# sonoisa/code2vec

Hardware: AMD Instinct MI355X
Metric: path_contexts_per_sec (higher is better)
Workload: dtype bf16; 1 GPU; model=code2vec-top11, global_batch=1024, seq_len=200, parallelism=dp1, terminal_vocab=360632, label_vocab=72416, embed=100, encode=100

## Files before the change

code2vec_amd/ops/csrc/bindings.cpp:

```cpp

#include <torch/extension.h>

#include <ATen/hip/HIPContext.h>
#include <c10/hip/HIPStream.h>
#include <hip/hip_runtime.h>

#include <map>

#define CHK(x) TORCH_CHECK(x, #x)
#define CHK_CONTIG(t) TORCH_CHECK((t).is_contiguous(), #t " must be contiguous")
#define CHK_CUDA(t) TORCH_CHECK((t).is_cuda(), #t " must be on GPU")
#define CHK_DT(t, dt) TORCH_CHECK((t).scalar_type() == dt, #t " dtype mismatch")

extern "C" {
void launch_gather_concat_fwd(const int*, const int*, const int*, const void*,
                              const void*, void*, long, int, int, int,
                              hipStream_t);
void launch_gather_concat_bwd(const int*, const int*, const int*, const void*,
                              float*, float*, long, int, int, hipStream_t);
void launch_embed_scatter_sorted(const int*, const long*, const void*, float*,
                                 void*, unsigned char*, long, long, int, int,
                                 int, int, int, hipStream_t);
void launch_embed_scatter_heavy(const int*, const long*, const int*,
                                const void*, float*, long, long, int, int,
                                int, int, int, hipStream_t);
void launch_adam_table_bf16(void*, const void*, const long*, int*, const int*,
                            float*, float*, float*, float*, long, int, long,
                            long, long, int, int, int, int, const double*,
                            float, float, float, float, float, int,
                            hipStream_t);
long group_tables_partials(long, long);
void launch_group_tables(const int*, const int*, const int*, long, int, int,
                         int*, int*, int*, int*, int*, int*, long*, int*,
                         long*, hipStream_t);
void launch_embed_scatter_heavy_pair(const int*, const long*, const int*,
                                     float*, int, const int*, const long*,
                                     const int*, float*, int, const void*,
                                     long, int, int, hipStream_t);
void launch_clear_i32_pair(int*, long, int*, long, hipStream_t);
void launch_count_indices(const int*, int*, long, hipStream_t);
void launch_cast_clear_rows(float*, const int*, unsigned char*, void*, long,
                            int, hipStream_t);
void launch_scatter_group(const int*, int*, int*, long*, long, hipStream_t);
void launch_exclusive_scan(const int*, int*, int*, long, hipStream_t);
size_t cub_exclusive_scan_temp_bytes(long);
void launch_cub_exclusive_scan(const int*, int*, void*, size_t, long,
                               hipStream_t);
void launch_combiner_fwd(const void*, const void*, const float*, const float*,
                         void*, void*, float*, float*, long, int, int, int,
                         float, unsigned long long,
                         const unsigned long long*, int, hipStream_t);
int launch_combiner_fwd_scores(const void*, const void*, const float*,
                               const float*, void*, void*, float*, float*,
                               long, int, int, int, float, unsigned long long,
                               const unsigned long long*, int, const float*,
                               float*, hipStream_t);
void launch_bump_u64(void*, unsigned long long, hipStream_t);
void launch_gather_combiner_fwd(const int*, const int*, const int*,
                                const void*, const void*, int, int,
                                const void*, const float*, const float*,
                                void*, void*, float*, float*, long, int, int,
                                int, float, unsigned long long,
                                const unsigned long long*, hipStream_t);
void launch_wgrad_gather(const int*, const int*, const int*, const void*,
                         const void*, int, int, const void*, float*, long,
                         int, int, int, hipStream_t);
void launch_combiner_bwd(const void*, const void*, const void*, const float*,
                         const float*, const float*, const float*, void*,
                         float*, float*, long, int, int, float, hipStream_t);
void launch_combiner_bwd_recompute(const float*, const float*, const void*,
                                   int, const float*, int, const void*,
                                   const void*, const float*, const float*,
                                   const float*, const float*, void*, float*,
                                   float*, long, int, float, hipStream_t);
void launch_attention_fwd(const void*, const float*, const int*, float*,
                          void*, float*, int, int, int, int, hipStream_t);
void launch_attention_bwd(const void*, int, const float*, const void*,
                          const float*, const int*, const float*, void*,
                          float*, float*, int, int, int, int, int,
                          hipStream_t);
int attention_stream_supported(int, int);
void launch_attention_fwd_scores(const void*, const float*, const int*,
                                 float*, void*, float*, int, int, int, int,
                                 hipStream_t);
void launch_attention_bwd_compact_reg(const void*, int, const float*,
                                      const void*, const int*, const float*,
                                      float*, float*, int, int, int, int, int,
                                      hipStream_t);
int attention_packed_chunk();
void launch_attention_packed_fwd(const void*, const float*, const int*,
                                 const int*, float*, void*, float*, long, long,
                                 int, int, hipStream_t);
void launch_attention_packed_bwd(const void*, int, const float*, const void*,
                                 const float*, const int*, const int*,
                                 const float*, void*, float*, int*, float*,
                                 long, long, int, int, hipStream_t);
void launch_combiner_bwd_recompute_packed(
    const float*, const float*, const void*, int, const float*, const int*,
    long, const void*, const void*, const float*, const float*, const float*,
    const float*, void*, float*, float*, long, int, float, hipStream_t);
void launch_slab_sum2_f32(const float*, const float*, float*, float*, int,
                          int, hipStream_t);
void launch_loss_reduce(const float*, float*, float*, int, hipStream_t);
void launch_wgrad_reduce(const float*, void*, int, int, int, hipStream_t);
void launch_lsm_nll_fwd(const void*, const long*, const float*, float*,
                        float*, int, long, hipStream_t);
void launch_lsm_nll_bwd(const void*, const long*, const float*, const float*,
                        const float*, const float*, void*, int, long,
                        hipStream_t);
bool launch_wgrad_pipe(const void*, const void*, float*, long, int, int, int,
                       int, hipStream_t);
void launch_wgrad(const void*, const void*, float*, long, int, int, int,
                  hipStream_t);
void launch_dgrad(const void*, const void*, void*, long, int, int,
                  hipStream_t);
void launch_head_wgrad(const void*, const void*, void*, long, long, int,
                       hipStream_t);
// ... 1257 lines not shown
  CHK_CUDA(sorted_idx); CHK_CONTIG(sorted_idx);
  CHK_DT(sorted_idx, torch::kInt32);
  CHK_DT(dtable, torch::kFloat32); CHK_CONTIG(dtable);
  TORCH_CHECK(dtable.dim() == 2, "dtable must be [T, S]");
  const long T = dtable.size(0);
  const int S = dtable.size(1);
  check_table_record(perm, counts, gout, T, S, M, KP, off0, off1);
  TORCH_CHECK(sorted_idx.numel() == perm.numel(), "sorted_idx/perm sizes");
  TORCH_CHECK(S % 2 == 0 && S <= 512 && KP % 2 == 0 && off0 % 2 == 0 &&
                  off1 % 2 == 0, "embed_scatter_heavy: S/KP/offset alignment");
  TORCH_CHECK(thr >= 32, "embed_scatter_heavy: thr must be >= 32");
  launch_embed_scatter_heavy(sorted_idx.data_ptr<int>(),
                             perm.data_ptr<long>(), counts.data_ptr<int>(),
                             gout.data_ptr(), dtable.data_ptr<float>(),
                             perm.numel(), M, (int)KP, S, (int)off0,
                             (int)off1, (int)thr, cur_stream());
}

static void adam_table_bf16_impl(
    torch::Tensor p, torch::Tensor gout, torch::Tensor perm,
    torch::Tensor counts, torch::Tensor cursor, torch::Tensor scratch,
    torch::Tensor master, torch::Tensor m, torch::Tensor v,
    torch::Tensor bc_pow, int64_t M, int64_t KP, int64_t off0, int64_t off1,
    int64_t thr, double lr, double b1, double b2, double eps, double wd,
    bool clear_counts) {
  CHK_CUDA(p); CHK_CONTIG(p); CHK_DT(p, torch::kBFloat16);
  TORCH_CHECK(p.dim() == 2, "p must be [T, S]");
  const long T = p.size(0);
  const int S = p.size(1);
  check_table_record(perm, counts, gout, T, S, M, KP, off0, off1);
  CHK_CONTIG(cursor); CHK_DT(cursor, torch::kInt32);
  TORCH_CHECK(cursor.numel() >= T, "cursor shorter than T");
  CHK_DT(scratch, torch::kFloat32); CHK_CONTIG(scratch);
  CHK_DT(master, torch::kFloat32); CHK_CONTIG(master);
  CHK_DT(m, torch::kFloat32); CHK_CONTIG(m);
  CHK_DT(v, torch::kFloat32); CHK_CONTIG(v);
  CHK_DT(bc_pow, torch::kFloat64);
  const long n = T * S;
  TORCH_CHECK(scratch.numel() == n && master.numel() == n &&
                  m.numel() == n && v.numel() == n, "state sizes");
  TORCH_CHECK(S % 4 == 0 && KP % 4 == 0 && off0 % 4 == 0 && off1 % 4 == 0,
              "adam_table_bf16: S, KP and offsets must be multiples of 4");
  TORCH_CHECK(n / 4 < (1L << 32), "adam_table_bf16: table too large");
  TORCH_CHECK(thr >= 32, "adam_table_bf16: thr must be >= 32");
  launch_adam_table_bf16(
      p.data_ptr(), gout.data_ptr(), perm.data_ptr<long>(),
      counts.data_ptr<int>(), cursor.data_ptr<int>(),
      scratch.data_ptr<float>(), master.data_ptr<float>(),
      m.data_ptr<float>(), v.data_ptr<float>(), T, S, counts.numel(),
      perm.numel(), M, (int)KP, (int)off0, (int)off1, (int)thr,
      (const double*)bc_pow.data_ptr(), (float)lr, (float)b1, (float)b2,
      (float)eps, (float)wd, clear_counts ? 1 : 0, cur_stream());
}

void adam_table_bf16(torch::Tensor p, torch::Tensor gout, torch::Tensor perm,
                     torch::Tensor counts, torch::Tensor cursor,
                     torch::Tensor scratch, torch::Tensor master,
                     torch::Tensor m, torch::Tensor v, torch::Tensor bc_pow,
                     int64_t M, int64_t KP, int64_t off0, int64_t off1,
                     int64_t thr, double lr, double b1, double b2, double eps,
                     double wd) {
  adam_table_bf16_impl(p, gout, perm, counts, cursor, scratch, master, m, v,
                       bc_pow, M, KP, off0, off1, thr, lr, b1, b2, eps, wd,
                       true);
}

void adam_table_bf16_keep_counts(
    torch::Tensor p, torch::Tensor gout, torch::Tensor perm,
    torch::Tensor counts, torch::Tensor cursor, torch::Tensor scratch,
    torch::Tensor master, torch::Tensor m, torch::Tensor v,
    torch::Tensor bc_pow, int64_t M, int64_t KP, int64_t off0, int64_t off1,
    int64_t thr, double lr, double b1, double b2, double eps, double wd) {
  adam_table_bf16_impl(p, gout, perm, counts, cursor, scratch, master, m, v,
                       bc_pow, M, KP, off0, off1, thr, lr, b1, b2, eps, wd,
                       false);
}


namespace {
struct GroupStream {
  hipStream_t side = nullptr;
  hipEvent_t ready = nullptr;
  hipEvent_t done = nullptr;
};
std::map<int, GroupStream>& group_streams() {
  static std::map<int, GroupStream> m;
  return m;
}
GroupStream& group_stream_for(int device) {
  auto& m = group_streams();
  auto it = m.find(device);
  if (it == m.end()) {
    GroupStream g;
    g.side = c10::hip::getStreamFromPool(false, device).stream();
    C10_HIP_CHECK(hipEventCreateWithFlags(&g.ready, hipEventDisableTiming));
    C10_HIP_CHECK(hipEventCreateWithFlags(&g.done, hipEventDisableTiming));
    it = m.emplace(device, g).first;
  }
  return it->second;
}
void check_i32(const torch::Tensor& t, long n, const char* what) {
  TORCH_CHECK(t.is_cuda() && t.is_contiguous() &&
                  t.scalar_type() == torch::kInt32 && t.numel() >= n,
              "group_tables: ", what, " must be contiguous int32 on the GPU "
              "with at least ", n, " elements");
}
}

bool group_tables(torch::Tensor starts, torch::Tensor paths,
                  torch::Tensor ends, torch::Tensor counts_t,
                  torch::Tensor counts_p, torch::Tensor cursor_t,
                  torch::Tensor cursor_p, torch::Tensor partial,
                  torch::Tensor sorted_t, torch::Tensor perm_t,
                  torch::Tensor sorted_p, torch::Tensor perm_p,
                  int64_t rows_t, int64_t rows_p, bool side_stream) {
  const long M = starts.numel();
  TORCH_CHECK(M > 0 && 2 * M < (1L << 31), "group_tables: bad entry count");
  TORCH_CHECK(rows_t > 0 && rows_p > 0 && rows_t < (1L << 31) &&
                  rows_p < (1L << 31), "group_tables: bad histogram length");
  check_i32(starts, M, "starts"); check_i32(paths, M, "paths");
  check_i32(ends, M, "ends");
  TORCH_CHECK(paths.numel() == M && ends.numel() == M,
              "group_tables: starts/paths/ends sizes differ");
  check_i32(counts_t, rows_t, "counts_t"); check_i32(counts_p, rows_p, "counts_p");
  check_i32(cursor_t, rows_t, "cursor_t"); check_i32(cursor_p, rows_p, "cursor_p");
  check_i32(partial, group_tables_partials(rows_t, rows_p), "partial");
  check_i32(sorted_t, 2 * M, "sorted_t"); check_i32(sorted_p, M, "sorted_p");
  CHK_CUDA(perm_t); CHK_CONTIG(perm_t); CHK_DT(perm_t, torch::kInt64);
  CHK_CUDA(perm_p); CHK_CONTIG(perm_p); CHK_DT(perm_p, torch::kInt64);
  TORCH_CHECK(perm_t.numel() >= 2 * M && perm_p.numel() >= M,
              "group_tables: perm buffers too short");

  auto cur = at::hip::getCurrentHIPStream();
  hipStream_t launch_on = cur.stream();
  bool on_side = false;
  GroupStream* gs = nullptr;
  if (side_stream) {
    hipStreamCaptureStatus cap = hipStreamCaptureStatusNone;
    C10_HIP_CHECK(hipStreamIsCapturing(cur.stream(), &cap));
    if (cap == hipStreamCaptureStatusNone) {
      gs = &group_stream_for(cur.device_index());
      C10_HIP_CHECK(hipEventRecord(gs->ready, cur.stream()));
      C10_HIP_CHECK(hipStreamWaitEvent(gs->side, gs->ready, 0));
      launch_on = gs->side;
      on_side = true;
    }
  }
  launch_group_tables(
      starts.data_ptr<int>(), paths.data_ptr<int>(), ends.data_ptr<int>(), M,
      (int)rows_t, (int)rows_p, counts_t.data_ptr<int>(),
      counts_p.data_ptr<int>(), cursor_t.data_ptr<int>(),
      cursor_p.data_ptr<int>(), partial.data_ptr<int>(),
      sorted_t.data_ptr<int>(), perm_t.data_ptr<long>(),
      sorted_p.data_ptr<int>(), perm_p.data_ptr<long>(), launch_on);
  if (on_side) C10_HIP_CHECK(hipEventRecord(gs->done, gs->side));
  return on_side;
}

void group_tables_wait() {
  auto cur = at::hip::getCurrentHIPStream();
  auto& m = group_streams();
  auto it = m.find(cur.device_index());
  TORCH_CHECK(it != m.end(), "group_tables_wait: no side-stream grouping");
  C10_HIP_CHECK(hipStreamWaitEvent(cur.stream(), it->second.done, 0));
}

int64_t group_tables_partials_len(int64_t rows_t, int64_t rows_p) {
  return group_tables_partials(rows_t, rows_p);
}

void embed_scatter_heavy_pair(torch::Tensor sorted_t, torch::Tensor perm_t,
                              torch::Tensor counts_t, torch::Tensor dtable_t,
                              torch::Tensor sorted_p, torch::Tensor perm_p,
                              torch::Tensor counts_p, torch::Tensor dtable_p,
                              torch::Tensor gout, int64_t M, int64_t KP,
                              int64_t thr) {
  CHK_DT(dtable_t, torch::kFloat32); CHK_CONTIG(dtable_t);
  CHK_DT(dtable_p, torch::kFloat32); CHK_CONTIG(dtable_p);
  TORCH_CHECK(dtable_t.dim() == 2 && dtable_p.dim() == 2,
              "dtable must be [T, S]");
  const int St = dtable_t.size(1), Sp = dtable_p.size(1);
  check_table_record(perm_t.narrow(0, 0, 2 * M), counts_t, gout,
                     dtable_t.size(0), St, M, KP, 0, St + Sp);
  check_table_record(perm_p.narrow(0, 0, M), counts_p, gout,
                     dtable_p.size(0), Sp, M, KP, St, St);
  check_i32(sorted_t, 2 * M, "sorted_t"); check_i32(sorted_p, M, "sorted_p");
  TORCH_CHECK(St % 2 == 0 && Sp % 2 == 0 && St <= 512 && Sp <= 512 &&
                  KP % 2 == 0, "embed_scatter_heavy_pair: S/KP alignment");
  TORCH_CHECK(thr >= 32, "embed_scatter_heavy_pair: thr must be >= 32");
  launch_embed_scatter_heavy_pair(
      sorted_t.data_ptr<int>(), perm_t.data_ptr<long>(),
      counts_t.data_ptr<int>(), dtable_t.data_ptr<float>(), St,
      sorted_p.data_ptr<int>(), perm_p.data_ptr<long>(),
      counts_p.data_ptr<int>(), dtable_p.data_ptr<float>(), Sp,
      gout.data_ptr(), M, (int)KP, (int)thr, cur_stream());
}

void clear_i32_pair(torch::Tensor a, torch::Tensor b) {
  check_i32(a, 0, "a"); check_i32(b, 0, "b");
  launch_clear_i32_pair(a.data_ptr<int>(), a.numel(), b.data_ptr<int>(),
                        b.numel(), cur_stream());
}

void adam_step_f32(torch::Tensor p, torch::Tensor g, torch::Tensor m,
                   torch::Tensor v, torch::Tensor bc_pow, double lr,
                   double b1, double b2, double eps, double wd) {
  CHK_CUDA(p); CHK_DT(p, torch::kFloat32); CHK_DT(g, torch::kFloat32);
  CHK_DT(bc_pow, torch::kFloat64);
  launch_adam_f32(p.data_ptr<float>(), g.data_ptr<float>(),
                  m.data_ptr<float>(), v.data_ptr<float>(), p.numel(),
                  (const double*)bc_pow.data_ptr(), (float)lr, (float)b1,
                  (float)b2, (float)eps, (float)wd, cur_stream());
}

void adam_step_f32_multi(std::vector<torch::Tensor> ps,
                         std::vector<torch::Tensor> gs,
                         std::vector<torch::Tensor> ms,
                         std::vector<torch::Tensor> vs,
                         torch::Tensor bc_pow, double lr, double b1,
                         double b2, double eps, double wd) {
  const int n = (int)ps.size();
  TORCH_CHECK(n >= 1 && n <= 8, "adam_step_f32_multi: 1..8 tensors");
  TORCH_CHECK((int)gs.size() == n && (int)ms.size() == n &&
              (int)vs.size() == n, "adam_step_f32_multi: list sizes");
  CHK_DT(bc_pow, torch::kFloat64);
  float* pp[8]; const float* gp[8]; float* mp[8]; float* vp[8]; long ns[8];
  for (int t = 0; t < n; ++t) {
    CHK_CUDA(ps[t]); CHK_CONTIG(ps[t]); CHK_DT(ps[t], torch::kFloat32);
    CHK_CONTIG(gs[t]); CHK_DT(gs[t], torch::kFloat32);
    TORCH_CHECK(ps[t].numel() == gs[t].numel() &&
                ps[t].numel() == ms[t].numel() &&
                ps[t].numel() == vs[t].numel(), "sizes");
    pp[t] = ps[t].data_ptr<float>();
    gp[t] = gs[t].data_ptr<float>();
    mp[t] = ms[t].data_ptr<float>();
    vp[t] = vs[t].data_ptr<float>();
    ns[t] = ps[t].numel();
  }
  launch_adam_f32_multi(pp, gp, mp, vp, ns, n,
                        (const double*)bc_pow.data_ptr(), (float)lr,
                        (float)b1, (float)b2, (float)eps, (float)wd,
                        cur_stream());
}

PYBIND11_MODULE(TORCH_EXTENSION_NAME, m) {
  m.def("gather_concat_fwd", &gather_concat_fwd);
  m.def("gather_concat_bwd", &gather_concat_bwd);
  m.def("embed_scatter_sorted", &embed_scatter_sorted);
  m.def("group_by_index", &group_by_index);
  m.def("cast_clear_rows", &cast_clear_rows);
  m.def("combiner_fwd", &combiner_fwd);
  m.def("gather_combiner_fwd", &gather_combiner_fwd);
  m.def("wgrad_gather", &wgrad_gather);
  m.def("combiner_bwd", &combiner_bwd);
  m.def("attention_fwd", &attention_fwd);
  m.def("attention_bwd", &attention_bwd);
  m.def("attention_fwd_cvb", &attention_fwd_cvb);
  m.def("attention_bwd_compact", &attention_bwd_compact);
  m.def("combiner_fwd_scores", &combiner_fwd_scores);
  m.def("attention_stream_ok", &attention_stream_ok);
  m.def("attention_fwd_scores", &attention_fwd_scores);
  m.def("attention_bwd_compact_reg", &attention_bwd_compact_reg);
  m.def("attention_pool_packed", &attention_pool_packed);
  m.def("combiner_bwd_recompute", &combiner_bwd_recompute);
  m.def("attention_packed_bwd_compact", &attention_packed_bwd_compact);
  m.def("attention_packed_bwd", &attention_packed_bwd);
  m.def("combiner_bwd_recompute_packed", &combiner_bwd_recompute_packed);
  m.def("slab_sum2_f32", &slab_sum2_f32);
  m.def("loss_reduce", &loss_reduce);
  m.def("wgrad_reduce", &wgrad_reduce);
  m.def("logsoftmax_nll_fwd", &logsoftmax_nll_fwd);
  m.def("logsoftmax_nll_bwd", &logsoftmax_nll_bwd);
  m.def("wgrad", &wgrad);
  m.def("wgrad_pipe", &wgrad_pipe);
  m.def("colsum_bf16", &colsum_bf16);
  m.def("head_fwd", &head_fwd);
  m.def("head_fwd_img", &head_fwd_img);
  m.def("swizzle_a", &swizzle_a);
  m.def("logsoftmax_nll_finalize", &logsoftmax_nll_finalize);
  m.def("lsm_partial", &lsm_partial);
  m.def("head_wgrad", &head_wgrad);
  m.def("head_dgrad", &head_dgrad);
  m.def("exclusive_scan", &exclusive_scan);
  m.def("cub_exclusive_scan", &cub_exclusive_scan);
  m.def("cub_scan_temp_bytes", &cub_scan_temp_bytes);
  m.def("head_bwd_prep", &head_bwd_prep);
  m.def("swizzle_cv", &swizzle_cv);
  m.def("row_max_argmax", &row_max_argmax);
  m.def("row_topk", &row_topk);
  m.def("sim_topk", &sim_topk);
  m.def("inv_rownorm", &inv_rownorm);
  m.def("rowscale", &rowscale);
  m.def("angular_fwd", &angular_fwd);
  m.def("angular_dcos", &angular_dcos);
  m.def("norm_project", &norm_project);
  m.def("head_bwd_dw", &head_bwd_dw);
  m.def("head_bwd_dcv", &head_bwd_dcv);
  m.def("head_bwd_dcv_rc", &head_bwd_dcv_rc);
  m.def("head_bwd_dw_pipe", &head_bwd_dw_pipe);
  m.def("head_bwd_dcv_pipe", &head_bwd_dcv_pipe);
  m.def("transpose_w", &transpose_w);
  m.def("dgrad2", &dgrad2);
  m.def("slab_sum_bf16", &slab_sum_bf16);
  m.def("slab_sum_f32", &slab_sum_f32);
  m.def("dgrad", &dgrad);
  m.def("adam_tick", &adam_tick);
  m.def("adam_step_bf16", &adam_step_bf16);
  m.def("adam_step_f32", &adam_step_f32);
  m.def("embed_scatter_heavy", &embed_scatter_heavy);
  m.def("adam_table_bf16", &adam_table_bf16);
  m.def("adam_step_f32_multi", &adam_step_f32_multi);
  m.def("adam_table_bf16_keep_counts", &adam_table_bf16_keep_counts);
  m.def("group_tables", &group_tables);
  m.def("group_tables_wait", &group_tables_wait);
  m.def("group_tables_partials_len", &group_tables_partials_len);
  m.def("embed_scatter_heavy_pair", &embed_scatter_heavy_pair);
  m.def("clear_i32_pair", &clear_i32_pair);
}
```

code2vec_amd/ops/csrc/index_group.hip:

```cpp

#include "common.h"
#include "scatter_heavy.h"

#define IG_BLOCK 256
#define IG_SCAN 1024

struct GroupTable {
  const int* idx0;
  const int* idx1;
  long split, N;
  int rows;
  int* counts;
  int* cursor;
  int* sorted_idx;
  long* perm;
};

template <int E>
__device__ __forceinline__ void load_entries(const GroupTable& t, long base,
                                             int (&v)[E]) {
#pragma unroll
  for (int j = 0; j < E; ++j) {
    const long e = base + j * IG_BLOCK + threadIdx.x;
    int x = -1;
// ... 51 lines not shown
      if (lane == leader) b = atomicAdd(&t.cursor[v[j]], (int)__popcll(m));
      pos[j] = __shfl(b, leader) + rank;
    } else if (v[j] > 1) {
      pos[j] = atomicAdd(&t.cursor[v[j]], 1);
    }
  }
#pragma unroll
  for (int j = 0; j < E; ++j) {
    if (v[j] >= 0 && (unsigned long)pos[j] < (unsigned long)t.N) {
      t.sorted_idx[pos[j]] = v[j];
      t.perm[pos[j]] = base + j * IG_BLOCK + threadIdx.x;
    }
  }
}

__device__ __forceinline__ int block_sum(int v, int* red) {
  const int lane = threadIdx.x & (WAVE - 1);
  const int wave = threadIdx.x / WAVE;
#pragma unroll
  for (int off = 32; off > 0; off >>= 1) v += __shfl_xor(v, off);
  __syncthreads();
  if (lane == 0) red[wave] = v;
  __syncthreads();
  return red[0] + red[1] + red[2] + red[3];
}

__global__ __launch_bounds__(IG_BLOCK) void group_scan_partials_kernel(
    const int* __restrict__ counts_t, int rows_t, const int* __restrict__ counts_p,
    int rows_p, int term_blocks, int* __restrict__ partial) {
  const bool is_path = (int)blockIdx.x >= term_blocks;
  const int* x = is_path ? counts_p : counts_t;
  const int n = is_path ? rows_p : rows_t;
  const int b0 = ((int)blockIdx.x - (is_path ? term_blocks : 0)) * IG_SCAN;
  int v = 0;
#pragma unroll
  for (int k = 0; k < IG_SCAN / IG_BLOCK; ++k) {
    const int i = b0 + k * IG_BLOCK + threadIdx.x;
    v += i < n ? x[i] : 0;
  }
  __shared__ int red[IG_BLOCK / WAVE];
  const int s = block_sum(v, red);
  if (threadIdx.x == 0) partial[blockIdx.x] = s;
}

__global__ __launch_bounds__(IG_BLOCK) void group_scan_apply_kernel(
    const int* __restrict__ counts_t, int rows_t, const int* __restrict__ counts_p,
    int rows_p, int term_blocks, const int* __restrict__ partial,
    int* __restrict__ cursor_t, int* __restrict__ cursor_p) {
  const bool is_path = (int)blockIdx.x >= term_blocks;
  const int* x = is_path ? counts_p : counts_t;
  int* out = is_path ? cursor_p : cursor_t;
  const int n = is_path ? rows_p : rows_t;
  const int seg0 = is_path ? term_blocks : 0;
  const int lb = (int)blockIdx.x - seg0;
  const int lane = threadIdx.x & (WAVE - 1);
  const int wave = threadIdx.x / WAVE;
  __shared__ int red[IG_BLOCK / WAVE];
  const int i0 = lb * IG_SCAN + threadIdx.x * 4;
  int c[4];
#pragma unroll
  for (int k = 0; k < 4; ++k) c[k] = i0 + k < n ? x[i0 + k] : 0;
  int pre = 0;
  for (int i = threadIdx.x; i < lb; i += IG_BLOCK) pre += partial[seg0 + i];
  const int prefix = block_sum(pre, red);
  const int tsum = c[0] + c[1] + c[2] + c[3];
  int inc = tsum;
#pragma unroll
  for (int off = 1; off < WAVE; off <<= 1) {
    const int up = __shfl_up(inc, off);
    if (lane >= off) inc += up;
  }
  __shared__ int wtot[IG_BLOCK / WAVE];
  if (lane == WAVE - 1) wtot[wave] = inc;
  __syncthreads();
  int run = prefix + inc - tsum;
  for (int w = 0; w < wave; ++w) run += wtot[w];
#pragma unroll
  for (int k = 0; k < 4; ++k) {
    if (i0 + k < n) out[i0 + k] = run;
    run += c[k];
  }
}

struct HeavyTable {
  const int* sorted_idx;
  const long* perm;
  const int* counts;
  float* dtable;
  long N;
  int S, off0, off1;
};

template <int NP>
__global__ __launch_bounds__(256) void embed_scatter_heavy_pair_kernel(
    HeavyTable term, HeavyTable path, int term_blocks,
    const bf16* __restrict__ gout, long M, int KP, int thr) {
  const bool is_path = (int)blockIdx.x >= term_blocks;
  const HeavyTable& t = is_path ? path : term;
  const long wid =
      (long)((int)blockIdx.x - (is_path ? term_blocks : 0)) *
          (blockDim.x / WAVE) + threadIdx.x / WAVE;
  scatter_heavy_chunk<NP>(wid, t.sorted_idx, t.perm, t.counts, gout, t.dtable,
                          t.N, M, KP, t.S, t.off0, t.off1, thr);
}

__global__ void clear_i32_pair_kernel(int* __restrict__ a, long na,
                                      int* __restrict__ b, long nb) {
  const long i = (long)blockIdx.x * blockDim.x + threadIdx.x;
  const long stride = (long)gridDim.x * blockDim.x;
  for (long j = i; j < na + nb; j += stride) {
    if (j < na) a[j] = 0;
    else b[j - na] = 0;
  }
}

extern "C" {

long group_tables_partials(long rows_t, long rows_p) {
  return (rows_t + IG_SCAN - 1) / IG_SCAN + (rows_p + IG_SCAN - 1) / IG_SCAN;
}

void launch_group_tables(const int* starts, const int* paths, const int* ends,
                         long M, int rows_t, int rows_p, int* counts_t,
                         int* counts_p, int* cursor_t, int* cursor_p,
                         int* partial, int* sorted_t, long* perm_t,
                         int* sorted_p, long* perm_p, hipStream_t stream) {
  if (M <= 0) return;
  GroupTable term = {starts, ends, M, 2 * M, rows_t, counts_t, cursor_t,
                     sorted_t, perm_t};
  GroupTable path = {paths, paths, M, M, rows_p, counts_p, cursor_p,
                     sorted_p, perm_p};
  static const char* ee = getenv("C2V_GROUP_E");
  const int E = ee && (atoi(ee) == 1 || atoi(ee) == 4) ? atoi(ee) : 2;
  const long tile = (long)IG_BLOCK * E;
  const int tb = (int)((2 * M + tile - 1) / tile);
  const int pb = (int)((M + tile - 1) / tile);
  const int st = (rows_t + IG_SCAN - 1) / IG_SCAN;
  const int sp = (rows_p + IG_SCAN - 1) / IG_SCAN;
#define IG_LAUNCH(kernel)                                                     \
  do {                                                                        \
    if (E == 1)                                                               \
      kernel<1><<<tb + pb, IG_BLOCK, 0, stream>>>(term, path, tb);            \
    else if (E == 2)                                                          \
      kernel<2><<<tb + pb, IG_BLOCK, 0, stream>>>(term, path, tb);            \
    else                                                                      \
      kernel<4><<<tb + pb, IG_BLOCK, 0, stream>>>(term, path, tb);            \
  } while (0)
  IG_LAUNCH(group_count_pair_kernel);
  group_scan_partials_kernel<<<st + sp, IG_BLOCK, 0, stream>>>(
      counts_t, rows_t, counts_p, rows_p, st, partial);
  group_scan_apply_kernel<<<st + sp, IG_BLOCK, 0, stream>>>(
      counts_t, rows_t, counts_p, rows_p, st, partial, cursor_t, cursor_p);
  IG_LAUNCH(group_scatter_pair_kernel);
#undef IG_LAUNCH
}

void launch_embed_scatter_heavy_pair(
    const int* sorted_t, const long* perm_t, const int* counts_t,
    float* dtable_t, int S_t, const int* sorted_p, const long* perm_p,
    const int* counts_p, float* dtable_p, int S_p, const void* gout, long M,
    int KP, int thr, hipStream_t stream) {
  if (M <= 0) return;
  HeavyTable term = {sorted_t, perm_t, counts_t, dtable_t, 2 * M,
                     S_t, 0, S_t + S_p};
  HeavyTable path = {sorted_p, perm_p, counts_p, dtable_p, M, S_p, S_t, S_t};
  const int wpb = 4;
  const int tb = (int)(((2 * M + 15) / 16 + wpb - 1) / wpb);
  const int pb = (int)(((M + 15) / 16 + wpb - 1) / wpb);
  const int S = S_t > S_p ? S_t : S_p;
#define HPCASE(n)                                                             \
  case n:                                                                     \
    embed_scatter_heavy_pair_kernel<n><<<tb + pb, 256, 0, stream>>>(          \
        term, path, tb, (const bf16*)gout, M, KP, thr);                       \
    break;
  switch ((S + 127) / 128) {
    HPCASE(1) HPCASE(2) HPCASE(3) HPCASE(4)
    default:
      printf("embed_scatter_heavy_pair: unsupported S=%d\n", S);
  }
#undef HPCASE
}

void launch_clear_i32_pair(int* a, long na, int* b, long nb,
                           hipStream_t stream) {
  const int block = 256;
  const long n = na + nb;
  const int grid = (int)min((n + block - 1) / block, (long)4096);
  clear_i32_pair_kernel<<<grid > 0 ? grid : 1, block, 0, stream>>>(a, na, b,
                                                                   nb);
}

}
```

code2vec_amd/ops/functional.py:

```python

from __future__ import annotations

import os
from typing import Optional

import torch

_FWD_EPI = int(os.environ.get("C2V_FWD_EPI", "1"))
_SCATTER_R = int(os.environ.get("C2V_SCATTER_R", "16"))
FUSE_GATHER_COMBINER = os.environ.get("C2V_FUSE") == "1"
_HEAD_FWD = os.environ.get("C2V_HEAD_FWD", "1") == "1"
_HEAD_FWD_MAXL = int(os.environ.get("C2V_HEAD_FWD_MAXL", "98304"))
_HF_AIMG = os.environ.get("C2V_HF_AIMG", "1") == "1"
_SCAN_CUB = os.environ.get("C2V_SCAN_CUB", "1") == "1"
_CUB_TEMP_BYTES: dict = {}
_HB_RC = os.environ.get("C2V_HB_RC", "0") == "1"
_HEAD_DGRAD = os.environ.get("C2V_HEAD_DGRAD", "1") == "1"
_DGRAD2 = os.environ.get("C2V_DGRAD2", "1") == "1"
FUSED_HEAD = os.environ.get("C2V_FUSED_HEAD", "1") == "1"
FUSED_CAP = os.environ.get("C2V_FUSED_CAP", "1") == "1"
_WGRAD_REDUCE = os.environ.get("C2V_WGRAD_REDUCE", "1") == "1"
_HB_PIPE = os.environ.get("C2V_HB_PIPE", "1") == "1"
_HB_PIPE_DW = _HB_PIPE and os.environ.get("C2V_HB_PIPE_DW", "1") == "1"
_HB_PIPE_DCV = _HB_PIPE and os.environ.get("C2V_HB_PIPE_DCV", "0") == "1"
# ... 212 lines not shown
            ext().embed_scatter_heavy_pair(
                t.sorted_idx, t.perm, t.counts,
                _scratch_f32("term", t.shape, param.device),
                p.sorted_idx, p.perm, p.counts,
                _scratch_f32("path", p.shape, param.device),
                rec.gout, rec.M, rec.KP, _TABLE_ADAM_HEAVY)
            pair.prepassed = True
        ext().adam_table_bf16_keep_counts(
            param, rec.gout, rec.perm, rec.counts, rec.cursor, scratch,
            master, m, v, bc_pow, rec.M, rec.KP, rec.off0, rec.off1,
            _TABLE_ADAM_HEAVY, lr, beta1, beta2, eps, weight_decay)
        pair.stepped.append(rec)
        if len(pair.stepped) == 2:
            ext().clear_i32_pair(t.counts, p.counts)
            pair.recs = {}
        rec._release()
        return
    if pair is None or not pair.prepassed:
        ext().embed_scatter_heavy(rec.sorted_idx, rec.perm, rec.counts,
                                  rec.gout, scratch, rec.M, rec.KP, rec.off0,
                                  rec.off1, _TABLE_ADAM_HEAVY)
    ext().adam_table_bf16(param, rec.gout, rec.perm, rec.counts, rec.cursor,
                          scratch, master, m, v, bc_pow, rec.M, rec.KP,
                          rec.off0, rec.off1, _TABLE_ADAM_HEAVY, lr, beta1,
                          beta2, eps, weight_decay)
    rec._release()


class _TableGrouping:

    __slots__ = ("ticket", "index_tensors", "tables", "on_side", "M",
                 "shapes", "keys")


_group_state = {"outstanding": None, "next_ticket": 1}


def _grouping_applies(term_key, path_key) -> bool:
    return all(k is not None and k in OWNED_GRAD_KEYS
               and k in DEFERRED_GRAD_KEYS and k in EARLY_GRAD_CALLBACKS
               for k in (term_key, path_key))


def _launch_table_grouping(starts, paths, ends, term_w, path_w,
                           row_capacity=None):
    if row_capacity is not None and starts.numel() > row_capacity:
        raise ValueError(
            f"packed batch has {starts.numel()} rows, over the row capacity "
            f"{row_capacity} its scratch was sized for")
    if not (_GROUP_TABLES and starts.is_cuda and term_w.requires_grad
            and path_w.requires_grad
            and _grouping_applies(term_w.data_ptr(), path_w.data_ptr())
            and starts.dtype == paths.dtype == ends.dtype == torch.int32
            and starts.is_contiguous() and paths.is_contiguous()
            and ends.is_contiguous() and starts.numel() > 0):
        return None
    retire_table_grouping()
    dev = starts.device
    M = starts.numel()
    g = _TableGrouping()
    g.tables = {}
    bufs = {}
    for tag, rows, n in (("term", term_w.shape[0] + 1, 2 * M),
                         ("path", path_w.shape[0] + 1, M)):
        counts = _scratch_i32(f"counts_{tag}", rows, dev)
        stale = _PENDING_DEFERRED.get(counts.data_ptr())
        if stale is not None:
            discard_deferred(stale)
        cursor = _scratch_i32(f"cursor_{tag}", rows, dev, zero=False)
        if row_capacity is None:
            sorted_idx = _scratch_i32(f"gsorted_{tag}", n, dev, zero=False)
            perm = _scratch_i64(f"gperm_{tag}", n, dev)
        else:
            cap = (n // M) * int(row_capacity)
            sorted_idx = _scratch_i32(f"gsorted_cap_{tag}", cap, dev,
                                      zero=False)[:n]
            perm = _scratch_i64(f"gperm_cap_{tag}", cap, dev)[:n]
        g.tables[tag] = (sorted_idx, perm, counts, cursor)
        bufs[tag] = rows
    spart = _scratch_i32(
        "gscanp", int(ext().group_tables_partials_len(bufs["term"],
                                                      bufs["path"])),
        dev, zero=False)
    st, sp = g.tables["term"], g.tables["path"]
    g.on_side = bool(ext().group_tables(
        starts, paths, ends, st[2], sp[2], st[3], sp[3], spart, st[0], st[1],
        sp[0], sp[1], bufs["term"], bufs["path"], _GROUP_STREAM))
    g.index_tensors = (starts, paths, ends)
    g.M = M
    g.shapes = (tuple(term_w.shape), tuple(path_w.shape))
    g.keys = (term_w.data_ptr(), path_w.data_ptr())
    g.ticket = _group_state["next_ticket"]
    _group_state["next_ticket"] += 1
    _group_state["outstanding"] = g
    return g.ticket


def _adopt_table_grouping(ticket, M, term_shape, path_shape, term_key,
                          path_key):
    g = _group_state["outstanding"]
    if g is None:
        return None
    if (ticket is None or g.ticket != ticket or g.M != M
            or g.shapes != (tuple(term_shape), tuple(path_shape))
            or g.keys != (term_key, path_key)
            or not _grouping_applies(term_key, path_key)):
        retire_table_grouping()
        return None
    _group_state["outstanding"] = None
    if g.on_side:
        ext().group_tables_wait()
    return g


def retire_table_grouping() -> None:
    g = _group_state["outstanding"]
    if g is None:
        return
    _group_state["outstanding"] = None
    if g.on_side:
        ext().group_tables_wait()
    for tag in ("term", "path"):
        g.tables[tag][2].zero_()


_scratch_cache = {}


def _scratch_f32(tag: str, shape, device) -> torch.Tensor:
    key = (tag, tuple(shape), str(device))
    buf = _scratch_cache.get(key)
    if buf is None:
        buf = torch.zeros(shape, dtype=torch.float32, device=device)
        _scratch_cache[key] = buf
    return buf


def _scratch_bf16(tag: str, shape, device) -> torch.Tensor:
    key = ("bf16", tag, tuple(shape), str(device))
    buf = _scratch_cache.get(key)
    if buf is None:
        buf = torch.empty(shape, dtype=torch.bfloat16, device=device)
        _scratch_cache[key] = buf
    return buf


def _scratch_i32(tag: str, n: int, device, zero: bool = True) -> torch.Tensor:
    key = ("i32", tag, n, str(device))
    buf = _scratch_cache.get(key)
    if buf is None:
        maker = torch.zeros if zero else torch.empty
        buf = maker(n, dtype=torch.int32, device=device)
        _scratch_cache[key] = buf
    return buf


def _scratch_i64(tag: str, n: int, device) -> torch.Tensor:
    key = ("i64", tag, n, str(device))
    buf = _scratch_cache.get(key)
    if buf is None:
        buf = torch.empty(n, dtype=torch.int64, device=device)
        _scratch_cache[key] = buf
    return buf


def _scratch_u8(tag: str, n: int, device) -> torch.Tensor:
    key = ("u8", tag, n, str(device))
    buf = _scratch_cache.get(key)
    if buf is None:
        buf = torch.empty(n, dtype=torch.uint8, device=device)
# ... 968 lines not shown
```

Measured before the change: 193.6 million path-contexts/s.

## Replace index grouping with two-level bucket radix partition

Embedding indices are now grouped with a two-level partition instead of the old count, scan and scatter pass over the full row histogram. Each tile builds a per-block histogram over coarse row buckets, a single kernel turns those into bucket offsets, and entries are partitioned into a temporary buffer. A per-bucket finish kernel then does the fine sort in LDS, which should avoid global atomics and the scan over a histogram with hundreds of thousands of rows. The change needs extra scratch memory, adds more kernel launches, and hot rows 0 and 1 take a special path.

After: 198.9 million path-contexts/s (median of 6 runs). 1.03x the previous value.

```diff
diff --git a/code2vec_amd/ops/csrc/bindings.cpp b/code2vec_amd/ops/csrc/bindings.cpp
--- a/code2vec_amd/ops/csrc/bindings.cpp
+++ b/code2vec_amd/ops/csrc/bindings.cpp
@@ -30,9 +30,10 @@
                             float, float, float, float, float, int,
                             hipStream_t);
 long group_tables_partials(long, long);
+long group_tables_tmp(long, long, long);
 void launch_group_tables(const int*, const int*, const int*, long, int, int,
                          int*, int*, int*, int*, int*, int*, long*, int*,
-                         long*, hipStream_t);
+                         long*, int*, hipStream_t);
 void launch_embed_scatter_heavy_pair(const int*, const long*, const int*,
                                      float*, int, const int*, const long*,
                                      const int*, float*, int, const void*,
@@ -1456,6 +1457,7 @@
   hipStream_t side = nullptr;
   hipEvent_t ready = nullptr;
   hipEvent_t done = nullptr;
+  torch::Tensor tmp;
 };
 std::map<int, GroupStream>& group_streams() {
   static std::map<int, GroupStream> m;
@@ -1487,7 +1489,8 @@
                   torch::Tensor cursor_p, torch::Tensor partial,
                   torch::Tensor sorted_t, torch::Tensor perm_t,
                   torch::Tensor sorted_p, torch::Tensor perm_p,
-                  int64_t rows_t, int64_t rows_p, bool side_stream) {
+                  int64_t rows_t, int64_t rows_p, bool side_stream,
+                  c10::optional<torch::Tensor> tmp) {
   const long M = starts.numel();
   TORCH_CHECK(M > 0 && 2 * M < (1L << 31), "group_tables: bad entry count");
   TORCH_CHECK(rows_t > 0 && rows_p > 0 && rows_t < (1L << 31) &&
@@ -1520,13 +1523,29 @@
       on_side = true;
     }
   }
+  const long tmp_len = group_tables_tmp(M, rows_t, rows_p);
+  torch::Tensor scratch;
+  if (tmp.has_value()) {
+    scratch = *tmp;
+    check_i32(scratch, tmp_len, "tmp");
+    TORCH_CHECK((uintptr_t)scratch.data_ptr() % 8 == 0,
+                "group_tables: tmp must be 8-byte aligned");
+  } else {
+    scratch = torch::empty({tmp_len}, starts.options());
+    if (on_side) {
+      if (gs->tmp.defined())
+        C10_HIP_CHECK(hipStreamWaitEvent(cur.stream(), gs->done, 0));
+      gs->tmp = scratch;
+    }
+  }
   launch_group_tables(
       starts.data_ptr<int>(), paths.data_ptr<int>(), ends.data_ptr<int>(), M,
       (int)rows_t, (int)rows_p, counts_t.data_ptr<int>(),
       counts_p.data_ptr<int>(), cursor_t.data_ptr<int>(),
       cursor_p.data_ptr<int>(), partial.data_ptr<int>(),
       sorted_t.data_ptr<int>(), perm_t.data_ptr<long>(),
-      sorted_p.data_ptr<int>(), perm_p.data_ptr<long>(), launch_on);
+      sorted_p.data_ptr<int>(), perm_p.data_ptr<long>(),
+      scratch.data_ptr<int>(), launch_on);
   if (on_side) C10_HIP_CHECK(hipEventRecord(gs->done, gs->side));
   return on_side;
 }
@@ -1541,6 +1560,10 @@
 
 int64_t group_tables_partials_len(int64_t rows_t, int64_t rows_p) {
   return group_tables_partials(rows_t, rows_p);
+}
+
+int64_t group_tables_tmp_len(int64_t M, int64_t rows_t, int64_t rows_p) {
+  return group_tables_tmp(M, rows_t, rows_p);
 }
 
 void embed_scatter_heavy_pair(torch::Tensor sorted_t, torch::Tensor perm_t,
@@ -1685,7 +1708,13 @@
   m.def("adam_table_bf16", &adam_table_bf16);
   m.def("adam_step_f32_multi", &adam_step_f32_multi);
   m.def("adam_table_bf16_keep_counts", &adam_table_bf16_keep_counts);
-  m.def("group_tables", &group_tables);
+  m.def("group_tables", &group_tables, py::arg("starts"), py::arg("paths"),
+        py::arg("ends"), py::arg("counts_t"), py::arg("counts_p"),
+        py::arg("cursor_t"), py::arg("cursor_p"), py::arg("partial"),
+        py::arg("sorted_t"), py::arg("perm_t"), py::arg("sorted_p"),
+        py::arg("perm_p"), py::arg("rows_t"), py::arg("rows_p"),
+        py::arg("side_stream"), py::arg("tmp") = py::none());
+  m.def("group_tables_tmp_len", &group_tables_tmp_len);
   m.def("group_tables_wait", &group_tables_wait);
   m.def("group_tables_partials_len", &group_tables_partials_len);
   m.def("embed_scatter_heavy_pair", &embed_scatter_heavy_pair);
diff --git a/code2vec_amd/ops/csrc/index_group.hip b/code2vec_amd/ops/csrc/index_group.hip
--- a/code2vec_amd/ops/csrc/index_group.hip
+++ b/code2vec_amd/ops/csrc/index_group.hip
@@ -157,6 +157,267 @@
   }
 }
 
+#define IG_MAXB 2048
+#define IG_FIN_BLOCK 512
+#define IG_FIN_U 4
+
+__device__ __forceinline__ int group_column(int v, int logr, int nbx) {
+  const int c = 2 + (v >> logr);
+  return c < nbx ? c : nbx - 1;
+}
+
+template <int E>
+__global__ __launch_bounds__(IG_BLOCK) void group_bucket_count_kernel(
+    GroupTable term, GroupTable path, int term_blocks, int logr,
+    int* __restrict__ mat_t, int nbx_t, int* __restrict__ mat_p, int nbx_p) {
+  const bool is_path = (int)blockIdx.x >= term_blocks;
+  const GroupTable& t = is_path ? path : term;
+  const int lb = (int)blockIdx.x - (is_path ? term_blocks : 0);
+  const int nbx = is_path ? nbx_p : nbx_t;
+  int* row = (is_path ? mat_p : mat_t) + (long)lb * nbx;
+  const int lane = threadIdx.x & (WAVE - 1);
+  __shared__ int hist[IG_MAXB + 2];
+  int v[E];
+  load_entries<E>(t, (long)lb * (IG_BLOCK * E), v);
+  for (int c = threadIdx.x; c < nbx; c += IG_BLOCK) hist[c] = 0;
+  __syncthreads();
+#pragma unroll
+  for (int j = 0; j < E; ++j) {
+    const unsigned long long m0 = __ballot(v[j] == 0);
+    const unsigned long long m1 = __ballot(v[j] == 1);
+    if (v[j] > 1) {
+      atomicAdd(&hist[group_column(v[j], logr, nbx)], 1);
+    } else if (v[j] >= 0) {
+      const unsigned long long m = v[j] == 0 ? m0 : m1;
+      if (lane == __ffsll((long long)m) - 1)
+        atomicAdd(&hist[v[j]], (int)__popcll(m));
+    }
+  }
+  __syncthreads();
+  for (int c = threadIdx.x; c < nbx; c += IG_BLOCK) row[c] = hist[c];
+}
+
+__global__ __launch_bounds__(1024) void group_bucket_offsets_kernel(
+    int* __restrict__ mat_t, int blocks_t, int nbx_t, int* __restrict__ bbase_t,
+    int* __restrict__ mat_p, int blocks_p, int nbx_p,
+    int* __restrict__ bbase_p) {
+  const bool is_path = blockIdx.x != 0;
+  int* mat = is_path ? mat_p : mat_t;
+  int* bbase = is_path ? bbase_p : bbase_t;
+  const int nblk = is_path ? blocks_p : blocks_t;
+  const int nbx = is_path ? nbx_p : nbx_t;
+  constexpr int CPT = (IG_MAXB + 2 + 1023) / 1024;
+  __shared__ int part[4][IG_MAXB + 2];
+  __shared__ int wtot[1024 / WAVE];
+  const int g = threadIdx.x >> 8, cl = threadIdx.x & 255;
+  const int lane = threadIdx.x & (WAVE - 1), wave = threadIdx.x / WAVE;
+  const int per = (nblk + 3) / 4;
+  const int r0 = min(g * per, nblk), r1 = min(r0 + per, nblk);
+  for (int c = cl; c < nbx; c += 256) {
+    int s = 0;
+#pragma unroll 8
+    for (int b = r0; b < r1; ++b) s += mat[(long)b * nbx + c];
+    part[g][c] = s;
+  }
+  __syncthreads();
+  int tot[CPT], tsum = 0;
+#pragma unroll
+  for (int j = 0; j < CPT; ++j) {
+    const int c = threadIdx.x * CPT + j;
+    tot[j] = c < nbx ? part[0][c] + part[1][c] + part[2][c] + part[3][c] : 0;
+    tsum += tot[j];
+  }
+  int inc = tsum;
+#pragma unroll
+  for (int off = 1; off < WAVE; off <<= 1) {
+    const int up = __shfl_up(inc, off);
+    if (lane >= off) inc += up;
+  }
+  if (lane == WAVE - 1) wtot[wave] = inc;
+  __syncthreads();
+  int run = inc - tsum;
+  for (int w = 0; w < wave; ++w) run += wtot[w];
+#pragma unroll
+  for (int j = 0; j < CPT; ++j) {
+    const int c = threadIdx.x * CPT + j;
+    if (c < nbx) {
+      bbase[c] = run;
+      if (c == nbx - 1) bbase[nbx] = run + tot[j];
+      int acc = run;
+#pragma unroll
+      for (int q = 0; q < 4; ++q) {
+        const int x = part[q][c];
+        part[q][c] = acc;
+        acc += x;
+      }
+    }
+    run += tot[j];
+  }
+  __syncthreads();
+  for (int c = cl; c < nbx; c += 256) {
+    int acc = part[g][c];
+    for (int b = r0; b < r1; b += 8) {
+      int x[8];
+#pragma unroll
+      for (int q = 0; q < 8; ++q)
+        x[q] = b + q < r1 ? mat[(long)(b + q) * nbx + c] : 0;
+#pragma unroll
+      for (int q = 0; q < 8; ++q) {
+        if (b + q < r1) mat[(long)(b + q) * nbx + c] = acc;
+        acc += x[q];
+      }
+    }
+  }
+}
+
+template <int E>
+__global__ __launch_bounds__(IG_BLOCK) void group_partition_kernel(
+    GroupTable term, GroupTable path, int term_blocks, int logr,
+    const int* __restrict__ mat_t, int nbx_t, int2* __restrict__ tmp_t,
+    const int* __restrict__ mat_p, int nbx_p, int2* __restrict__ tmp_p) {
+  const bool is_path = (int)blockIdx.x >= term_blocks;
+  const GroupTable& t = is_path ? path : term;
+  const int lb = (int)blockIdx.x - (is_path ? term_blocks : 0);
+  const int nbx = is_path ? nbx_p : nbx_t;
+  const int* row = (is_path ? mat_p : mat_t) + (long)lb * nbx;
+  int2* tmp = is_path ? tmp_p : tmp_t;
+  const long base = (long)lb * (IG_BLOCK * E);
+  const int lane = threadIdx.x & (WAVE - 1);
+  __shared__ int cur[IG_MAXB + 2];
+  int v[E];
+  load_entries<E>(t, base, v);
+  for (int c = threadIdx.x; c < nbx; c += IG_BLOCK) cur[c] = row[c];
+  __syncthreads();
+  int pos[E];
+#pragma unroll
+  for (int j = 0; j < E; ++j) {
+    const unsigned long long m0 = __ballot(v[j] == 0);
+    const unsigned long long m1 = __ballot(v[j] == 1);
+    pos[j] = -1;
+    if (v[j] > 1) {
+      pos[j] = atomicAdd(&cur[group_column(v[j], logr, nbx)], 1);
+    } else if (v[j] >= 0) {
+      const unsigned long long m = v[j] == 0 ? m0 : m1;
+      const int leader = __ffsll((long long)m) - 1;
+      const int rank = (int)__popcll(m & ((1ull << lane) - 1));
+      int b = 0;
+      if (lane == leader) b = atomicAdd(&cur[v[j]], (int)__popcll(m));
+      pos[j] = __shfl(b, leader) + rank;
+    }
+  }
+#pragma unroll
+  for (int j = 0; j < E; ++j) {
+    if (v[j] >= 0 && (unsigned long)pos[j] < (unsigned long)t.N) {
+      const long e = base + j * IG_BLOCK + threadIdx.x;
+      if (v[j] <= 1) {
+        t.sorted_idx[pos[j]] = v[j];
+        t.perm[pos[j]] = e;
+      } else {
+        tmp[pos[j]] = make_int2(v[j], (int)e);
+      }
+    }
+  }
+}
+
+template <int LOGR, int NC>
+__global__ __launch_bounds__(IG_FIN_BLOCK) void group_bucket_finish_kernel(
+    GroupTable term, GroupTable path, int term_buckets,
+    const int* __restrict__ bbase_t, const int2* __restrict__ tmp_t,
+    const int* __restrict__ bbase_p, const int2* __restrict__ tmp_p) {
+  constexpr int R = 1 << LOGR;
+  constexpr int RPT = R / IG_FIN_BLOCK;
+  const bool is_path = (int)blockIdx.x >= term_buckets;
+  const GroupTable& t = is_path ? path : term;
+  const int k = (int)blockIdx.x - (is_path ? term_buckets : 0);
+  const int* bbase = is_path ? bbase_p : bbase_t;
+  const int2* tmp = is_path ? tmp_p : tmp_t;
+  const int lane = threadIdx.x & (WAVE - 1), wave = threadIdx.x / WAVE;
+  const int copy = lane & (NC - 1);
+  const int row0 = k << LOGR;
+  __shared__ int h[R * NC];
+  __shared__ int wtot[IG_FIN_BLOCK / WAVE];
+  const int N = (int)t.N;
+  const int b0 = min(max(bbase[2 + k], 0), N);
+  const int b1 = min(max(bbase[3 + k], b0), N);
+  for (int i = threadIdx.x; i < R * NC; i += IG_FIN_BLOCK) h[i] = 0;
+  __syncthreads();
+  for (long i0 = b0; i0 < b1; i0 += IG_FIN_BLOCK * IG_FIN_U) {
+    int2 x[IG_FIN_U];
+#pragma unroll
+    for (int j = 0; j < IG_FIN_U; ++j) {
+      const long i = i0 + j * IG_FIN_BLOCK + threadIdx.x;
+      x[j] = i < b1 ? tmp[i] : make_int2(-1, 0);
+    }
+#pragma unroll
+    for (int j = 0; j < IG_FIN_U; ++j) {
+      const int r = x[j].x - row0;
+      if ((unsigned)r < (unsigned)R) atomicAdd(&h[r * NC + copy], 1);
+    }
+  }
+  __syncthreads();
+  int rc[RPT], tsum = 0;
+#pragma unroll
+  for (int j = 0; j < RPT; ++j) {
+    const int r = threadIdx.x * RPT + j;
+    int s = 0;
+#pragma unroll
+    for (int c = 0; c < NC; ++c) s += h[r * NC + c];
+    rc[j] = s;
+    tsum += s;
+  }
+  int inc = tsum;
+#pragma unroll
+  for (int off = 1; off < WAVE; off <<= 1) {
+    const int up = __shfl_up(inc, off);
+    if (lane >= off) inc += up;
+  }
+  if (lane == WAVE - 1) wtot[wave] = inc;
+  __syncthreads();
+  int run = b0 + inc - tsum;
+  for (int w = 0; w < wave; ++w) run += wtot[w];
+#pragma unroll
+  for (int j = 0; j < RPT; ++j) {
+    const int r = threadIdx.x * RPT + j;
+    int acc = run;
+#pragma unroll
+    for (int c = 0; c < NC; ++c) {
+      const int x = h[r * NC + c];
+      h[r * NC + c] = acc;
+      acc += x;
+    }
+    run += rc[j];
+    int cnt = rc[j], end = run;
+    if (k == 0 && r <= 1) {
+      cnt = bbase[r + 1] - bbase[r];
+      end = bbase[r + 1];
+    }
+    if (row0 + r < t.rows) {
+      t.counts[row0 + r] = cnt;
+      t.cursor[row0 + r] = end;
+    }
+  }
+  __syncthreads();
+  for (long i0 = b0; i0 < b1; i0 += IG_FIN_BLOCK * IG_FIN_U) {
+    int2 x[IG_FIN_U];
+#pragma unroll
+    for (int j = 0; j < IG_FIN_U; ++j) {
+      const long i = i0 + j * IG_FIN_BLOCK + threadIdx.x;
+      x[j] = i < b1 ? tmp[i] : make_int2(-1, 0);
+    }
+#pragma unroll
+    for (int j = 0; j < IG_FIN_U; ++j) {
+      const int r = x[j].x - row0;
+      if ((unsigned)r < (unsigned)R) {
+        const int pos = atomicAdd(&h[r * NC + copy], 1);
+        if (pos >= b0 && pos < b1) {
+          t.sorted_idx[pos] = x[j].x;
+          t.perm[pos] = x[j].y;
+        }
+      }
+    }
+  }
+}
+
 struct HeavyTable {
   const int* sorted_idx;
   const long* perm;
@@ -191,20 +452,83 @@
 
 extern "C" {
 
+#define IG_MIN_R 1024
+#define IG_MIN_TILE 1024
+
 long group_tables_partials(long rows_t, long rows_p) {
-  return (rows_t + IG_SCAN - 1) / IG_SCAN + (rows_p + IG_SCAN - 1) / IG_SCAN;
+  return (rows_t + IG_SCAN - 1) / IG_SCAN + (rows_p + IG_SCAN - 1) / IG_SCAN +
+         8;
+}
+
+long group_tables_tmp(long M, long rows_t, long rows_p) {
+  const long bt = (2 * M + IG_MIN_TILE - 1) / IG_MIN_TILE;
+  const long bp = (M + IG_MIN_TILE - 1) / IG_MIN_TILE;
+  const long ct = (rows_t + IG_MIN_R - 1) / IG_MIN_R + 2;
+  const long cp = (rows_p + IG_MIN_R - 1) / IG_MIN_R + 2;
+  return 6 * M + bt * ct + bp * cp;
+}
+
+static int group_env(const char* name, int a, int b, int c, int dflt) {
+  const char* e = getenv(name);
+  const int x = e ? atoi(e) : dflt;
+  return x == a || x == b || x == c ? x : dflt;
 }
 
 void launch_group_tables(const int* starts, const int* paths, const int* ends,
                          long M, int rows_t, int rows_p, int* counts_t,
                          int* counts_p, int* cursor_t, int* cursor_p,
                          int* partial, int* sorted_t, long* perm_t,
-                         int* sorted_p, long* perm_p, hipStream_t stream) {
+                         int* sorted_p, long* perm_p, int* tmp,
+                         hipStream_t stream) {
   if (M <= 0) return;
   GroupTable term = {starts, ends, M, 2 * M, rows_t, counts_t, cursor_t,
                      sorted_t, perm_t};
   GroupTable path = {paths, paths, M, M, rows_p, counts_p, cursor_p,
                      sorted_p, perm_p};
+  const int R = group_env("C2V_GROUP_R", 1024, 2048, 4096, 2048);
+  const int logr = R == 1024 ? 10 : R == 2048 ? 11 : 12;
+  const int nb_t = (int)(((long)rows_t + R - 1) >> logr);
+  const int nb_p = (int)(((long)rows_p + R - 1) >> logr);
+  if (tmp != nullptr && group_env("C2V_GROUP_SORT", 0, 1, 1, 1) == 1 &&
+      nb_t <= IG_MAXB && nb_p <= IG_MAXB) {
+    const int tile = group_env("C2V_GROUP_TILE", 1024, 2048, 4096, 4096);
+    const int tb = (int)((2 * M + tile - 1) / tile);
+    const int pb = (int)((M + tile - 1) / tile);
+    const int nbx_t = nb_t + 2, nbx_p = nb_p + 2;
+    int2* tmp_t = (int2*)tmp;
+    int2* tmp_p = tmp_t + 2 * M;
+    int* mat_t = tmp + 6 * M;
+    int* mat_p = mat_t + (long)tb * nbx_t;
+    int* bbase_t = partial;
+    int* bbase_p = partial + nbx_t + 1;
+#define IG_TILE_LAUNCH(kernel, ...)                                           \
+  do {                                                                        \
+    if (tile == 1024)                                                         \
+      kernel<4><<<tb + pb, IG_BLOCK, 0, stream>>>(term, path, tb, logr,       \
+                                                  __VA_ARGS__);               \
+    else if (tile == 2048)                                                    \
+      kernel<8><<<tb + pb, IG_BLOCK, 0, stream>>>(term, path, tb, logr,       \
+                                                  __VA_ARGS__);               \
+    else                                                                      \
+      kernel<16><<<tb + pb, IG_BLOCK, 0, stream>>>(term, path, tb, logr,      \
+                                                   __VA_ARGS__);              \
+  } while (0)
+    IG_TILE_LAUNCH(group_bucket_count_kernel, mat_t, nbx_t, mat_p, nbx_p);
+    group_bucket_offsets_kernel<<<2, 1024, 0, stream>>>(
+        mat_t, tb, nbx_t, bbase_t, mat_p, pb, nbx_p, bbase_p);
+    IG_TILE_LAUNCH(group_partition_kernel, mat_t, nbx_t, tmp_t, mat_p, nbx_p,
+                   tmp_p);
+#undef IG_TILE_LAUNCH
+#define IG_FIN_LAUNCH(lr, nc)                                                 \
+  group_bucket_finish_kernel<lr, nc>                                          \
+      <<<nb_t + nb_p, IG_FIN_BLOCK, 0, stream>>>(term, path, nb_t, bbase_t,   \
+                                                 tmp_t, bbase_p, tmp_p)
+    if (logr == 10) IG_FIN_LAUNCH(10, 8);
+    else if (logr == 11) IG_FIN_LAUNCH(11, 8);
+    else IG_FIN_LAUNCH(12, 4);
+#undef IG_FIN_LAUNCH
+    return;
+  }
   static const char* ee = getenv("C2V_GROUP_E");
   const int E = ee && (atoi(ee) == 1 || atoi(ee) == 4) ? atoi(ee) : 2;
   const long tile = (long)IG_BLOCK * E;
diff --git a/code2vec_amd/ops/functional.py b/code2vec_amd/ops/functional.py
--- a/code2vec_amd/ops/functional.py
+++ b/code2vec_amd/ops/functional.py
@@ -318,10 +318,18 @@
         "gscanp", int(ext().group_tables_partials_len(bufs["term"],
                                                       bufs["path"])),
         dev, zero=False)
+    tmp_n = int(ext().group_tables_tmp_len(M, bufs["term"], bufs["path"]))
+    if row_capacity is None:
+        gtmp = _scratch_i32("gtmp", tmp_n, dev, zero=False)
+    else:
+        gtmp = _scratch_i32(
+            "gtmp_cap", int(ext().group_tables_tmp_len(
+                int(row_capacity), bufs["term"], bufs["path"])),
+            dev, zero=False)[:tmp_n]
     st, sp = g.tables["term"], g.tables["path"]
     g.on_side = bool(ext().group_tables(
         starts, paths, ends, st[2], sp[2], st[3], sp[3], spart, st[0], st[1],
-        sp[0], sp[1], bufs["term"], bufs["path"], _GROUP_STREAM))
+        sp[0], sp[1], bufs["term"], bufs["path"], _GROUP_STREAM, gtmp))
     g.index_tensors = (starts, paths, ends)
     g.M = M
     g.shapes = (tuple(term_w.shape), tuple(path_w.shape))
```
